# joshspeagle/brutus

Hardware: AMD Instinct MI355X
Metric: stars/sec at 750k-model x 12-band grid; achieved HBM GB/s vs peak (higher is better)
Workload: dtype f64; 1 GPU; configs[1]: 750k-model x 12-band grid, Av-only solve (rvlim=(3.32,3.32)), no parallax; grid = synth.make_mist_like_grid (lattice-ordered like the MIST grid files); grid_generator=mist_like, nmodel=750000, nfilt=12, sub_batch=128, selected_models_last_sub_batch=44670752, streams_per_gpu=3, parallelism=stars sharded, 1 rank(s), no data-path collective

## Files before the change

### brutus_amd/csrc/brutus_kernels.hip

```cpp

#include <hip/hip_runtime.h>
#include <math.h>
#include <stdint.h>
#include <string.h>

#include <atomic>
#include <vector>

#include "../../include/brutus_amd.h"
#include "../../include/brutus_amd_debug.h"

#include "host.hpp"
#include "common.hpp"
#include "fastmath.hpp"
#include "grid_kernels.hpp"
#include "fit_kernels.hpp"
#include "fit2_kernels.hpp"
#include "cut_kernels.hpp"

namespace {

struct ResBlock {
    enum { SELECTED, DERIVED, CANDIDATES, NTOTALS = 4, NUNCONV = 4, NCTR = 8, ZEROED = NUNCONV + NCTR };
    int64_t *totals;
    int32_t *k1, *k2, *n_unconv, *ctr;
    ResBlock(int64_t *base, int nstar) : totals(base), k1((int32_t *)(base + NTOTALS)), k2(k1 + nstar),
                                         n_unconv(k2 + nstar), ctr(n_unconv + NUNCONV) {}
    static size_t bytes(int nstar) { return sizeof(int64_t) * NTOTALS + sizeof(int32_t) * (2 * (size_t)nstar + ZEROED); }
};

struct Workspace {
    Planes pl;
    StarPrep *stars;
    double *part;
    double *vmax_lnlp;
    int32_t *k1;
    int32_t *k2;
    int32_t *n_unconv;
    int64_t *counts;
    int64_t *offsets;
    int32_t *ids;
    int32_t *ids2;
    int32_t *ctr;
    int32_t *hot;
    int64_t *res;
    int32_t *kfix;
    double *thr_cull, *maxsurv, *thr_sel;
    int32_t *surv_idx;
    int64_t *surv_off;
    int64_t *coffsets;
    int64_t *dcounts, *doffsets;
    int64_t *der_off;
    int32_t *wbase_surv, *wbase_der;
    ItemGeom *items_surv, *items_der;
    int32_t *bandn;
    unsigned long long *mask, *dmask;
    unsigned long long *smask;
    double *step_st, *lnprob_st;
    Star32 *s32;
    float *lnlp32, *lnpr32;
    float *part32, *st32;
    int32_t *status, *ids_all;
    double *nomA, *nomB, *candS;
    float *aud;
    StarPrep *stars_tmp;
    size_t part_doubles;
    size_t bytes;
};

Workspace carve(char *base, int64_t nmodel, int nstar, bool fit) {
    Workspace w{};
    Carver cv(base);
    const size_t pairs = (size_t)nstar * (size_t)nmodel;
    const int64_t ntile = pad_models(nmodel) / TILE;
    w.pl.nmodel = nmodel;
    w.stars = (StarPrep *)cv.take(sizeof(StarPrep) * nstar);
    w.part_doubles = (size_t)ntile * (size_t)(nstar * 2 * KCAP > 1024 ? nstar * 2 * KCAP : 1024);
    w.part = (double *)cv.take(sizeof(double) * w.part_doubles);
    w.stars_tmp = (StarPrep *)cv.take(sizeof(StarPrep));
    w.vmax_lnlp = (double *)cv.take(sizeof(double) * nstar);
    w.k1 = (int32_t *)cv.take(sizeof(int32_t) * nstar);
    w.k2 = (int32_t *)cv.take(sizeof(int32_t) * nstar);
    w.n_unconv = (int32_t *)cv.take(sizeof(int32_t) * 4);
    w.counts = (int64_t *)cv.take(sizeof(int64_t) * nstar * NCHUNK);
    w.offsets = (int64_t *)cv.take(sizeof(int64_t) * nstar * NCHUNK);
    if (!fit) {
        w.pl.lnlp = (double *)cv.take_big(sizeof(double) * pairs);
        w.pl.step = (double *)cv.take_big(sizeof(double) * pairs);
    } else {
        w.ids = (int32_t *)cv.take(sizeof(int32_t) * nstar);
        w.ids2 = (int32_t *)cv.take(sizeof(int32_t) * nstar);
        w.res = (int64_t *)cv.take(ResBlock::bytes(nstar));
        if (base) {
            const ResBlock res(w.res, nstar);
            w.k1 = res.k1;
            w.k2 = res.k2;
            w.n_unconv = res.n_unconv;
            w.ctr = res.ctr;
        }
        w.kfix = (int32_t *)cv.take(sizeof(int32_t) * nstar);
        w.thr_cull = (double *)cv.take(sizeof(double) * nstar);
        w.maxsurv = (double *)cv.take(sizeof(double) * nstar);
        w.thr_sel = (double *)cv.take(sizeof(double) * nstar);
        w.surv_off = (int64_t *)cv.take(sizeof(int64_t) * (nstar + 1));
        w.der_off = (int64_t *)cv.take(sizeof(int64_t) * (nstar + 1));
        w.coffsets = (int64_t *)cv.take(sizeof(int64_t) * nstar * NCHUNK);
        w.dcounts = (int64_t *)cv.take(sizeof(int64_t) * nstar * NCHUNK);
        w.doffsets = (int64_t *)cv.take(sizeof(int64_t) * nstar * NCHUNK);
        w.wbase_surv = (int32_t *)cv.take(sizeof(int32_t) * ((size_t)NCHUNK * nstar + 1));
        w.wbase_der = (int32_t *)cv.take(sizeof(int32_t) * ((size_t)NCHUNK * nstar + 1));
        {
            const size_t nit = (size_t)nstar * ((size_t)(pad_models(nmodel) / TILE) + NCHUNK);
            w.items_surv = (ItemGeom *)cv.take(sizeof(ItemGeom) * nit);
            w.items_der = (ItemGeom *)cv.take(sizeof(ItemGeom) * nit);
        }
        w.bandn = (int32_t *)cv.take(sizeof(int32_t) * (size_t)NCHUNK * nstar);
        const size_t words = (size_t)nstar * (size_t)(pad_models(nmodel) / 64);
        w.mask = (unsigned long long *)cv.take_big(sizeof(unsigned long long) * words);
        w.dmask = (unsigned long long *)cv.take_big(sizeof(unsigned long long) * words);
        w.smask = (unsigned long long *)cv.take_big(sizeof(unsigned long long) * words);
        const size_t nblk2 = (size_t)(ntile + F2_T - 1) / F2_T;
        w.s32 = (Star32 *)cv.take(sizeof(Star32) * nstar);
        w.part32 = (float *)cv.take(sizeof(float) * nblk2 * nstar * NV32);
        w.hot = (int32_t *)cv.take(sizeof(int32_t) * nblk2 * nstar);
        w.st32 = (float *)cv.take(sizeof(float) * nstar * NV32);
        w.status = (int32_t *)cv.take(sizeof(int32_t) * nstar);
        w.ids_all = (int32_t *)cv.take(sizeof(int32_t) * nstar);
        w.nomA = (double *)cv.take(sizeof(double) * nstar);
        w.nomB = (double *)cv.take(sizeof(double) * nstar);
        w.candS = (double *)cv.take(sizeof(double) * nstar);
        w.aud = (float *)cv.take(sizeof(float) * nstar * 4);
        w.lnlp32 = (float *)cv.take_big(sizeof(float) * pairs);
        w.lnpr32 = (float *)cv.take_big(sizeof(float) * pairs);
        w.surv_idx = (int32_t *)cv.take_big(sizeof(int32_t) * pairs);
        w.step_st = (double *)cv.take_big(sizeof(double) * pairs);
        w.lnprob_st = (double *)cv.take_big(sizeof(double) * pairs);
    }
    w.bytes = align_big(cv.off) + (base ? 0 : (size_t)4 << 20);
    return w;
}

int make_params(const brutus_params *in, DevParams &p) {
    if (!in) return fail(BRUTUS_EINVAL, "params is NULL");
    if (!(in->init_thresh > 0.) || !(in->ltol_subthresh > 0.))
        return fail(BRUTUS_EINVAL, "thresholds must be positive");
    if (in->init_thresh > in->ltol_subthresh)
        return fail(BRUTUS_EINVAL,
                    "The initial threshold must be smaller than or equal to the "
                    "final threshold applied to be useful!");
    p.avmin = in->avlim[0];
    p.avmax = in->avlim[1];
    p.rvmin = in->rvlim[0];
    p.rvmax = in->rvlim[1];
    p.av_mean = in->av_gauss[0];
    p.av_ivar = 1. / (in->av_gauss[1] * in->av_gauss[1]);
    p.rv_mean = in->rv_gauss[0];
    p.rv_ivar = 1. / (in->rv_gauss[1] * in->rv_gauss[1]);
    p.mtol = 2.5 * in->ltol;
    p.ltol = in->ltol;
    p.ln_init = log(in->init_thresh);
    p.ln_sub = log(in->ltol_subthresh);
    p.ln_wt = in->wt_thresh > 0. ? log(in->wt_thresh) : -INFINITY;
    p.a_reg = 1. / (0.05 * 0.05);
    p.r_reg = 1. / (0.1 * 0.1);
    p.dim_prior = in->dim_prior ? 1 : 0;
    return 0;
}

template <int NB>
int probe_k1_deep(const float *grid, int64_t nmodel, int star, const DevParams &p, int max_iter,
                  Workspace &w, int32_t *k1_out, hipStream_t st, const double *av_init = nullptr,
                  const double *rv_init = nullptr) {
    const int64_t nmodel_pad = pad_models(nmodel);
    const int ntile = (int)(nmodel_pad / TILE);
    HIP_TRY(hipMemcpyAsync(w.stars_tmp, w.stars + star, sizeof(StarPrep), hipMemcpyDeviceToDevice, st));
    const int cap = (int)(w.part_doubles / ((size_t)ntile * 2));
    for (int kmax = 16;; kmax *= 2) {
        if (kmax > max_iter) kmax = max_iter;
        if (kmax > cap) kmax = cap;
        hipLaunchKernelGGL(k_mag_stats<NB>, dim3(ntile, 1), dim3(TILE), 0, st, grid, nmodel,
                           nmodel_pad, 1, w.stars_tmp, p, kmax, w.part, av_init, rv_init);
        hipLaunchKernelGGL(k_k1_deep_decide, dim3(1), dim3(256), 0, st, ntile, kmax, w.part,
                           p.ln_init, w.k1 + star);
        HIP_TRY(hipMemcpyAsync(k1_out, w.k1 + star, sizeof(int32_t), hipMemcpyDeviceToHost, st));
        HIP_TRY(hipStreamSynchronize(st));
        if (*k1_out > 0) return 0;
        if (kmax >= max_iter || kmax >= cap)
            return fail(BRUTUS_ENOCONV, "magnitude phase of star %d not converged after %d sweeps",
// ... 58 lines not shown
                           w.part, p.ln_sub, (double *)nullptr, w.k2, w.n_unconv);
        HIP_TRY(hipMemcpyAsync(&h_unconv, w.n_unconv, sizeof(int32_t), hipMemcpyDeviceToHost, st));
        HIP_TRY(hipStreamSynchronize(st));
        if (h_unconv == 0) break;
        if (iter >= max_iter)
            return fail(BRUTUS_ENOCONV, "flux phase not converged after %d iterations for %d star(s)",
                        iter, h_unconv);
        ++iter;
    }

    tm.begin("k_finalize");
    hipLaunchKernelGGL(k_finalize, dim3(ntile, nstar), blk, 0, st, nmodel, nstar, w.stars, p,
                       w.vmax_lnlp, w.pl);
    tm.end();
    if (h_k1) HIP_TRY(hipMemcpyAsync(h_k1, w.k1, sizeof(int32_t) * nstar, hipMemcpyDeviceToHost, st));
    if (h_k2) HIP_TRY(hipMemcpyAsync(h_k2, w.k2, sizeof(int32_t) * nstar, hipMemcpyDeviceToHost, st));
    HIP_TRY(hipGetLastError());
    return 0;
}

int dispatch_pipeline(int nb, const float *grid, int64_t nmodel, int nstar, const DevParams &p,
                      int max_iter, Workspace &w, int32_t *h_k1, int32_t *h_k2,
                      hipStream_t st, Timer &tm, const double *av_init, const double *rv_init) {
    int rc = 0;
    if (with_nb(nb, GridBands{}, [&](auto NB) {
            rc = run_pipeline<decltype(NB)::value>(grid, nmodel, nstar, p, max_iter, w, h_k1, h_k2, st, tm, av_init, rv_init);
        }))
        return rc;
    return fail(BRUTUS_EINVAL, "unsupported band count %d", nb);
}

constexpr int BRUTUS_RETRY_HOSTDRIVEN = -1000;
std::atomic<long long> g_fit_calls{0}, g_fit_retries{0};
constexpr int FS_TILES_PER_BLOCK = 8, PERSIST_BLOCKS = 4096, CONT_BLOCKS = 2048, TOP_BLOCKS = 1024;

struct FitCall {
    const float *grid;
    int64_t nmodel, nmodel_pad;
    int ntile, nblkx;
    int nfilt, nstar;
    DevParams p;
    int max_iter;
    Workspace w;
    RecPlanes rec;
    int64_t capacity;
    int32_t *d_rec_idx, *d_rec_slot;
    int64_t *d_rec_off;
    int32_t *h_k1, *h_k2;
    int64_t *h_counts;
    hipStream_t st;
    Timer tm;
    int flux_rounds = 4;
    bool list_fast = true;
    int list_run = -LIST_RUN;
    bool audited = false;
    float *aud = nullptr;
};

inline bool rv_pinned(const DevParams &p) { return p.rvmin == p.rvmax && p.rv_mean == p.rvmin; }

P32 make_p32(const DevParams &p, int nfilt) {
    return P32{(float)p.avmin, (float)p.avmax, (float)p.rvmin, (float)p.rvmax, (float)p.av_mean, (float)p.av_ivar,
               (float)p.rv_mean, (float)p.rv_ivar, (float)(p.mtol * 1.002 + 1e-4), (float)(p.mtol * 0.998 - 1e-4),
               p.dim_prior, nfilt};
}

template <int NB, bool RVF>
int launch_pre32(FitCall &c, const int32_t *list, int nrun, const int32_t *nrun_dev, int accept,
                 int32_t *ctr, bool two_sweeps) {
    constexpr int G = 4;
    const Workspace &w = c.w;
    const P32 q = make_p32(c.p, c.nfilt);
    const int use_mfma = env_int("BRUTUS_PRE32_MFMA", 0);
    const int min_stars = env_int("BRUTUS_PRE32_STAR_LANES_MIN", 32);
    const bool lanes_are_stars = brutus_i_pre32s_bands(NB) && two_sweeps && nrun >= min_stars &&
                                 env_int("BRUTUS_PRE32_STAR_LANES", 1) != 0;
    c.tm.begin("k_pre32");
    if (lanes_are_stars) {
        if (brutus_i_pre32s_launch(NB, use_mfma, RVF ? 1 : 0, c.grid, c.nmodel, c.nmodel_pad, c.nstar, nrun, list,
                                   w.s32, &q, w.lnlp32, w.lnpr32, w.part32, c.st))
            return fail(BRUTUS_EHIP, "star-lane float32 pass: launch failed");
    } else {
        hipLaunchKernelGGL((k_pre32<NB, RVF, G>), dim3(8 * ((c.nblkx + 7) / 8) * ((nrun + G - 1) / G)),
                           dim3(TILE), 0, c.st, c.grid, c.nmodel, c.nmodel_pad, c.nstar, nrun, list, w.s32, q,
                           w.kfix, c.ntile, w.lnlp32, w.lnpr32, w.part32, nrun_dev);
    }
    c.tm.end();
    hipLaunchKernelGGL(k_pre_decide, dim3(nrun), dim3(256), 0, c.st, c.nblkx, c.nstar, list, w.part32,
                       w.s32, (float)c.p.ln_init, RVF ? 1 : 0, w.kfix, accept, w.st32, w.k1, w.status,
                       w.nomA, ctr, w.ids2, w.ids, nrun_dev);
    HIP_TRY(hipGetLastError());
    return 0;
}

template <int NB, bool RVF>
int pre32_all_stars(FitCall &c) { return launch_pre32<NB, RVF>(c, c.w.ids_all, c.nstar, nullptr, 0, c.w.ctr, true); }
template <int NB, bool RVF>
int pre32_redo_on_device(FitCall &c) { return launch_pre32<NB, RVF>(c, c.w.ids, c.nstar, c.w.ctr + 1, 1, nullptr, false); }
template <int NB, bool RVF>
int pre32_host_list(FitCall &c, const std::vector<int32_t> &ids, const std::vector<int32_t> &kfix, int accept) {
    const int nrun = (int)ids.size();
    HIP_TRY(hipMemcpyAsync(c.w.ids, ids.data(), sizeof(int32_t) * nrun, hipMemcpyHostToDevice, c.st));
    HIP_TRY(hipMemcpyAsync(c.w.kfix, kfix.data(), sizeof(int32_t) * c.nstar, hipMemcpyHostToDevice, c.st));
    bool two_sweeps = true;
    if (!RVF)
        for (int k = 0; k < nrun && two_sweeps; ++k) two_sweeps = kfix[ids[k]] == 2;
// ... 56 lines not shown
    const Workspace &w = c.w;
    if (c.aud) HIP_TRY(hipMemsetAsync(w.aud, 0, sizeof(float) * c.nstar * 4, c.st));
    c.h_counts[0] = c.h_counts[1] = c.h_counts[2] = 0;
    hipLaunchKernelGGL(k_prep32, dim3(c.nstar), dim3(64), 0, c.st, c.nstar, w.stars,
                       (float)env_double("BRUTUS_EPS_SCALE", 1.0), c.p.dim_prior, w.s32,
                       CallInit{w.ids_all, w.kfix, w.k2, w.n_unconv, ResBlock::ZEROED});
    return 0;
}

template <int NB, bool RVF>
int classify_on_device(FitCall &c) {
    if (int rc = pre32_all_stars<NB, RVF>(c)) return rc;
    if (int rc = k1probe_device_list<NB, RVF>(c)) return rc;
    if (!RVF)
        if (int rc = pre32_redo_on_device<NB, RVF>(c)) return rc;
    return 0;
}

template <int NB, bool RVF>
int classify_on_host(FitCall &c) {
    Workspace &w = c.w;
    const int nstar = c.nstar;
    std::vector<int32_t> ids(nstar), kfix(nstar, 2), k1(nstar, 0), status(nstar, 0);
    for (int s = 0; s < nstar; ++s) ids[s] = s;
    if (int rc = pre32_host_list<NB, RVF>(c, ids, kfix, 0)) return rc;
    HIP_TRY(hipMemcpyAsync(k1.data(), w.k1, sizeof(int32_t) * nstar, hipMemcpyDeviceToHost, c.st));
    HIP_TRY(hipMemcpyAsync(status.data(), w.status, sizeof(int32_t) * nstar, hipMemcpyDeviceToHost, c.st));
    HIP_TRY(hipStreamSynchronize(c.st));
    std::vector<int32_t> probe, redo;
    for (int s = 0; s < nstar; ++s) {
        if (status[s] == 1) redo.push_back(s);
        if (status[s] == 2) probe.push_back(s);
    }
    if (!probe.empty()) {
        if (int rc = k1probe_host_list<NB, RVF>(c, probe)) return rc;
        HIP_TRY(hipMemcpyAsync(k1.data(), w.k1, sizeof(int32_t) * nstar, hipMemcpyDeviceToHost, c.st));
        HIP_TRY(hipStreamSynchronize(c.st));
        for (int s : probe) {
            if (k1[s] == 0)
                if (int rc = probe_k1_deep<NB>(c.grid, c.nmodel, s, c.p, c.max_iter, w, &k1[s], c.st)) return rc;
            if (k1[s] > c.max_iter)
                return fail(BRUTUS_ENOCONV, "magnitude phase of star %d needs %d sweeps (max_iter %d)", s,
                            k1[s], c.max_iter);
            kfix[s] = k1[s];
            if (!RVF && k1[s] != 2) redo.push_back(s);
        }
    }
    for (int s : redo) kfix[s] = k1[s];
    if (!redo.empty())
        if (int rc = pre32_host_list<NB, RVF>(c, redo, kfix, 1)) return rc;
    return 0;
}

template <int NB, bool RVF>
void cull_candidates(FitCall &c) {
    const Workspace &w = c.w;
    const int nstar = c.nstar;
    const dim3 blk(TILE);
    c.tm.begin("k_top");
    hipLaunchKernelGGL(k_hot_list, dim3(nstar), dim3(256), 0, c.st, c.nblkx, nstar, 0, w.part32, w.nomA,
                       (const double *)nullptr, w.s32, (double *)nullptr, w.part, w.hot, w.ctr + 4);
    hipLaunchKernelGGL((k_top1<NB, RVF>), dim3(TOP_BLOCKS), blk, 0, c.st, c.grid, c.nmodel, c.nmodel_pad, nstar,
                       w.stars, c.p, w.k1, c.ntile, 0, w.lnlp32, w.nomA, w.hot, w.ctr + 4, w.part, c.aud);
    c.tm.end();
    hipLaunchKernelGGL(k_top_decide, dim3(nstar), dim3(256), 0, c.st, c.nblkx, nstar, w.ids_all, 0, w.part,
                       w.s32, c.p.ln_init, (const double *)nullptr, w.thr_cull, w.candS);
    c.tm.begin("k_surv_compact");
    if (!c.list_fast)
        hipLaunchKernelGGL(k_cmp_count32, dim3(NCHUNK, nstar), blk, 0, c.st, c.nmodel, c.ntile, w.lnlp32, w.candS,
                           w.counts, w.smask);
    else if (c.nmodel % 4 == 0)
        hipLaunchKernelGGL(k_cmp_count32_live<true>, dim3(NCHUNK, nstar), blk, 0, c.st, c.nmodel, c.ntile, nstar,
                           w.lnlp32, w.part32, w.candS, w.counts, w.smask);
    else
        hipLaunchKernelGGL(k_cmp_count32_live<false>, dim3(NCHUNK, nstar), blk, 0, c.st, c.nmodel, c.ntile, nstar,
                           w.lnlp32, w.part32, w.candS, w.counts, w.smask);
    const OffsetsJob job{w.counts, w.coffsets, w.surv_off, w.wbase_surv, w.res + ResBlock::CANDIDATES};
    hipLaunchKernelGGL(k_offsets, dim3(2), dim3(OFF_T), 0, c.st, nstar, job, job);
    hipLaunchKernelGGL(k_items, dim3((NCHUNK * nstar + 255) / 256), dim3(256), 0, c.st, nstar, w.wbase_surv,
                       w.coffsets, w.surv_off, w.items_surv);
    hipLaunchKernelGGL(k_cmp_scatter, dim3(NCHUNK, nstar), blk, 0, c.st, c.nmodel, c.ntile, w.smask,
                       w.coffsets, (int64_t)nstar * c.nmodel, w.surv_idx);
    c.tm.end();
}

enum class Asked { HostAfterFirstFlux, DeviceCandidates, WholeCall };
int capacity_verdict(const FitCall &c, Asked when, int64_t ncand, int64_t nder) {
    int64_t *n = c.h_counts;
    if (when != Asked::WholeCall) {
        if (ncand <= c.capacity) return 0;
        n[1] = ncand;
        n[2] = when == Asked::HostAfterFirstFlux
                   ? 2 * ncand
                   : ncand + (nder > 0 ? nder : ncand);
        return fail(BRUTUS_ENOMEM, "record buffer too small: %lld candidate slots, capacity %lld",
                    (long long)ncand, (long long)c.capacity);
    }
    n[1] = ncand;
    n[2] = ncand + nder;
    if (n[2] > c.capacity)
        return fail(BRUTUS_ENOMEM, "record buffer too small: %lld slots needed, capacity %lld",
                    (long long)n[2], (long long)c.capacity);
    return 0;
}

template <int NB, bool RVF>
void flux_on_device(FitCall &c) {
    const Workspace &w = c.w;
    for (int r = 0; r <= c.flux_rounds; ++r) {
        c.tm.begin(r == 0 ? "k_fflux" : "k_fflux_cont");
        if (r == 0) fflux_open<NB, RVF>(c);
        else fflux_continue_device<NB, RVF>(c, r, w.n_unconv + ((r - 1) & 1));
        c.tm.end();
        hipLaunchKernelGGL(k_fflux_decide, dim3(c.nstar), dim3(256), 0, c.st, c.nstar, w.wbase_surv, w.part,
                           c.p.ln_sub, w.k2, w.maxsurv, w.n_unconv + (r & 1), w.ids, w.n_unconv + ((r + 1) & 1));
    }
}

template <int NB, bool RVF>
int flux_on_host(FitCall &c, int64_t *ncand) {
    const Workspace &w = c.w;
    const int nstar = c.nstar;
    HIP_TRY(hipMemcpyAsync(ncand, w.surv_off + nstar, sizeof(int64_t), hipMemcpyDeviceToHost, c.st));
    int32_t h_unconv = 0;
    int iter = 2;
    std::vector<int32_t> k2s(nstar), act;
    for (int first = 1;; first = 0) {
        HIP_TRY(hipMemsetAsync(w.n_unconv, 0, sizeof(int32_t), c.st));
        c.tm.begin(first ? "k_fflux" : "k_fflux_cont");
        if (first) fflux_open<NB, RVF>(c);
        else fflux_continue_host<NB, RVF>(c, (int)act.size());
        c.tm.end();
        hipLaunchKernelGGL(k_fflux_decide, dim3(nstar), dim3(256), 0, c.st, nstar, w.wbase_surv, w.part,
                           c.p.ln_sub, w.k2, w.maxsurv, w.n_unconv, (int32_t *)nullptr, (int32_t *)nullptr);
        HIP_TRY(hipMemcpyAsync(&h_unconv, w.n_unconv, sizeof(int32_t), hipMemcpyDeviceToHost, c.st));
        HIP_TRY(hipMemcpyAsync(k2s.data(), w.k2, sizeof(int32_t) * nstar, hipMemcpyDeviceToHost, c.st));
        HIP_TRY(hipStreamSynchronize(c.st));
        if (first)
            if (int rc = capacity_verdict(c, Asked::HostAfterFirstFlux, *ncand, 0)) return rc;
        if (h_unconv == 0) return 0;
        if (iter >= c.max_iter)
            return fail(BRUTUS_ENOCONV, "flux phase not converged after %d iterations for %d star(s)",
                        iter, h_unconv);
        ++iter;
        act.clear();
        for (int s = 0; s < nstar; ++s)
            if (k2s[s] >= 0) act.push_back(s);
        HIP_TRY(hipMemcpyAsync(w.ids, act.data(), sizeof(int32_t) * act.size(), hipMemcpyHostToDevice, c.st));
    }
}

template <int NB, bool RVF>
void select_and_derive(FitCall &c) {
    const Workspace &w = c.w;
    const int nstar = c.nstar;
    const dim3 blk(TILE);
    c.tm.begin("k_top");
    hipLaunchKernelGGL(k_hot_list, dim3(nstar), dim3(256), 0, c.st, c.nblkx, nstar, 1, w.part32,
                       (const double *)nullptr, w.maxsurv, w.s32, w.nomB, w.part, w.hot, w.ctr + 5);
    hipLaunchKernelGGL((k_top1<NB, RVF>), dim3(TOP_BLOCKS), blk, 0, c.st, c.grid, c.nmodel, c.nmodel_pad, nstar,
                       w.stars, c.p, w.k1, c.ntile, 1, w.lnpr32, w.nomB, w.hot, w.ctr + 5, w.part,
                       c.aud ? c.aud + nstar : nullptr);
    c.tm.end();
    hipLaunchKernelGGL(k_top_decide, dim3(nstar), dim3(256), 0, c.st, c.nblkx, nstar, w.ids_all, 1, w.part,
                       w.s32, c.p.ln_wt, w.maxsurv, w.thr_sel, (double *)nullptr);
    c.tm.begin("k_sel_classify");
    if (c.list_fast && c.nmodel % 4 == 0)
        hipLaunchKernelGGL(k_sel_classify_live, dim3(NCHUNK, nstar), blk, 0, c.st, c.nmodel, c.ntile, nstar, w.s32,
                           w.lnpr32, w.part32, w.candS, w.lnprob_st, w.surv_off, w.thr_sel, w.counts, w.mask, w.dcounts,
                           w.dmask, w.surv_idx, w.bandn);
    else
        hipLaunchKernelGGL(k_sel_classify, dim3(NCHUNK, nstar), blk, 0, c.st, c.nmodel, c.ntile, w.s32, w.lnpr32,
                           w.lnprob_st, w.surv_off, w.thr_sel, w.counts, w.mask, w.dcounts, w.dmask, w.surv_idx, w.bandn);
    c.tm.end();
    c.tm.begin("k_sel_band");
    hipLaunchKernelGGL((k_sel_band<NB, RVF>), dim3(NCHUNK / SB_C, nstar, SB_Z), blk, 0, c.st, c.grid, c.nmodel,
                       c.nmodel_pad, c.ntile, w.stars, c.p, w.k1, w.lnpr32, w.thr_sel, w.surv_idx, w.bandn,
                       w.counts, w.mask, w.dcounts, w.dmask, c.aud ? c.aud + 2 * nstar : nullptr);
    c.tm.end();
    c.tm.begin("k_select");
    const OffsetsJob sel{w.counts, w.offsets, c.d_rec_off, nullptr, w.res + ResBlock::SELECTED};
    const OffsetsJob der{w.dcounts, w.doffsets, w.der_off, w.wbase_der, w.res + ResBlock::DERIVED};
    hipLaunchKernelGGL(k_offsets, dim3(4), dim3(OFF_T), 0, c.st, nstar, sel, der);
    hipLaunchKernelGGL(k_items, dim3((NCHUNK * nstar + 255) / 256), dim3(256), 0, c.st, nstar, w.wbase_der,
                       w.doffsets, w.der_off, w.items_der);
    hipLaunchKernelGGL(k_rec_index, dim3(NCHUNK, nstar), blk, 0, c.st, c.nmodel, c.ntile, nstar, w.mask, w.dmask,
                       w.smask, w.offsets, w.doffsets, w.coffsets, w.surv_off, c.capacity, c.d_rec_idx,
                       c.d_rec_slot, w.surv_idx);
    c.tm.end();
    c.tm.begin("k_derive");
    hipLaunchKernelGGL((k_derive<NB, RVF>), dim3(PERSIST_BLOCKS), blk, 0, c.st, c.grid, c.nmodel_pad, nstar,
                       w.stars, c.p, w.k1, w.surv_idx, w.wbase_der, w.items_der, w.surv_off, c.rec, c.list_run);
    c.tm.end();
}

int read_results(FitCall &c, std::vector<int64_t> &h_res) {
    h_res.resize((ResBlock::bytes(c.nstar) + sizeof(int64_t) - 1) / sizeof(int64_t));
    HIP_TRY(hipMemcpyAsync(h_res.data(), c.w.res, ResBlock::bytes(c.nstar), hipMemcpyDeviceToHost, c.st));
    HIP_TRY(hipGetLastError());
    HIP_TRY(hipStreamSynchronize(c.st));
    const ResBlock res(h_res.data(), c.nstar);
    c.h_counts[0] = res.totals[ResBlock::SELECTED];
    if (c.h_k1) memcpy(c.h_k1, res.k1, sizeof(int32_t) * c.nstar);
    if (c.h_k2) memcpy(c.h_k2, res.k2, sizeof(int32_t) * c.nstar);
    return 0;
}

template <int NB, bool RVF>
int run_fit(FitCall &c, bool device_driven) {
    int64_t ncand = 0;
    std::vector<int64_t> h_res;
    if (int rc = start_call(c)) return rc;
    if (int rc = device_driven ? classify_on_device<NB, RVF>(c) : classify_on_host<NB, RVF>(c)) return rc;
    cull_candidates<NB, RVF>(c);
    if (device_driven)
        flux_on_device<NB, RVF>(c);
    else if (int rc = flux_on_host<NB, RVF>(c, &ncand))
        return rc;
    select_and_derive<NB, RVF>(c);
    if (int rc = read_results(c, h_res)) return rc;
    const ResBlock res(h_res.data(), c.nstar);
    const int64_t nder = res.totals[ResBlock::DERIVED];
    if (device_driven) {
        ncand = res.totals[ResBlock::CANDIDATES];
        if (int rc = capacity_verdict(c, Asked::DeviceCandidates, ncand, nder)) return rc;
        if (res.ctr[3] != 0 || res.n_unconv[c.flux_rounds & 1] != 0) return BRUTUS_RETRY_HOSTDRIVEN;
    }
    return capacity_verdict(c, Asked::WholeCall, ncand, nder);
}

int audit_verdict(const Workspace &w, int nstar, hipStream_t st) {
    std::vector<float> aud(4 * (size_t)nstar);
    std::vector<Star32> s32(nstar);
    HIP_TRY(hipMemcpyAsync(aud.data(), w.aud, sizeof(float) * aud.size(), hipMemcpyDeviceToHost, st));
    HIP_TRY(hipMemcpyAsync(s32.data(), w.s32, sizeof(Star32) * (size_t)nstar, hipMemcpyDeviceToHost, st));
    HIP_TRY(hipStreamSynchronize(st));
    static const char *what[3] = {"cull statistic", "first-cut statistic (maximum)", "first-cut statistic (band)"};
    for (int r = 0; r < 3; ++r)
        for (int s = 0; s < nstar; ++s)
            if (!(aud[(size_t)r * nstar + s] < s32[s].eps))
                return fail(BRUTUS_EPRECISION,
                            "float32 proof bound violated: star %d of the batch, %s: |float32 - float64| = %.3g "
                            "against eps = %.3g (BRUTUS_EPS_SCALE raises the bound; please report the input)",
                            s, what[r], (double)aud[(size_t)r * nstar + s], (double)s32[s].eps);
    return 0;
}

int dispatch_fit(int nb, FitCall &c) {
    const bool rvf = rv_pinned(c.p);
    const bool hostdriven = env_int("BRUTUS_FIT_HOSTDRIVEN", 0) != 0;
    const long long call_no = g_fit_calls.fetch_add(1);
    const int every = env_int("BRUTUS_AUDIT_EVERY", 64);
    c.audited = every > 0 && call_no % every == 0;
    c.aud = env_int("BRUTUS_AUDIT", 0) != 0 || c.audited ? c.w.aud : nullptr;
    c.flux_rounds = env_int("BRUTUS_FLUX_ROUNDS", 4);
    c.list_fast = env_int("BRUTUS_LIST_FAST", 1) != 0;
    c.list_run = env_int("BRUTUS_LIST_RUN", 0);
    if (c.list_run < 1 || c.list_run > 64) c.list_run = -LIST_RUN;
    if (brutus_i_pre32_layout(0) != (int)sizeof(Star32) || brutus_i_pre32_layout(1) != (int)sizeof(P32) ||
        brutus_i_pre32_layout(2) != F2_T || brutus_i_pre32_layout(3) != TILE || brutus_i_pre32_layout(4) != NV32)
        return fail(BRUTUS_EINVAL, "float32 pass: the library's translation units disagree on the Star32 / "
                                   "tile layout (built with different flags?)");
    int rc = 0;
    const bool built = with_nb(nb, FitBands{}, [&](auto NB) {
        constexpr int N = decltype(NB)::value;
        auto run = [&](bool device_driven) {
            return rvf ? run_fit<N, true>(c, device_driven) : run_fit<N, false>(c, device_driven);
        };
        rc = hostdriven ? BRUTUS_RETRY_HOSTDRIVEN : run(true);
        if (rc == BRUTUS_RETRY_HOSTDRIVEN) {
            if (!hostdriven) g_fit_retries.fetch_add(1);
            rc = run(false);
        }
        if (rc == 0 && c.audited) rc = audit_verdict(c.w, c.nstar, c.st);
    });
    if (built) return rc;
    if (nb > BRUTUS_MAX_FILT_FIT)
        return fail(BRUTUS_EINVAL, "brutus_fit_batch fits at most %d bands at once (%d given): take the full-grid "
                                   "outputs of brutus_loglike_batch and cut on them", BRUTUS_MAX_FILT_FIT, c.nfilt);
    return fail(BRUTUS_EINVAL, "unsupported band count %d", nb);
}

int check_common(int64_t nmodel, int nfilt, int nstar) {
    if (nmodel <= 0 || nmodel > (int64_t)1 << 31) return fail(BRUTUS_EINVAL, "bad nmodel");
    if (padded_nb(nfilt) < 0 || nfilt < 1)
        return fail(BRUTUS_EINVAL, "nfilt=%d unsupported (max %d)", nfilt, BRUTUS_MAX_FILT);
    if (nstar < 1 || nstar > BRUTUS_MAX_BATCH)
        return fail(BRUTUS_EINVAL, "nstar=%d outside [1, %d]", nstar, BRUTUS_MAX_BATCH);
    return 0;
}

int launch_prep(int nstar, int nfilt, const double *d_flux, const double *d_err,
                const uint8_t *d_mask, const double *d_par, const double *d_perr, int has_par,
                Workspace &w, int32_t *d_ndim, hipStream_t st) {
    hipLaunchKernelGGL(k_prep, dim3(nstar), dim3(64), 0, st, nstar, nfilt, d_flux,
                       d_err, d_mask, d_par, d_perr, (d_par && d_perr) ? has_par : 0, w.stars,
                       d_ndim);
    HIP_TRY(hipGetLastError());
    return 0;
}

void fix_k2(int32_t *h_k2, int nstar) {
    if (!h_k2) return;
    for (int s = 0; s < nstar; ++s)
        if (h_k2[s] < 0) h_k2[s] = -h_k2[s] - 1;
}

}

// ... 200 lines not shown
        tm.collect();
        return fail(BRUTUS_ENOMEM, "record buffer too small: %lld rows needed, capacity %lld",
                    (long long)(rec_base + total), (long long)capacity);
    }
    CutPlanes pl;
    pl.v[0] = d_lnl;
    pl.v[1] = d_chi2;
    pl.v[2] = d_scale;
    pl.v[3] = d_av;
    pl.v[4] = d_rv;
    for (int q = 0; q < 6; ++q) pl.v[5 + q] = d_icov + (size_t)q * nstar * nmodel;
    tm.begin("cut_scatter");
    if (vec)
        hipLaunchKernelGGL(k_cut_scatter<true>, grid, block, 0, st, nmodel, w.stride, span, nstar,
                           w.lnprob, w.thr, w.counts, w.offsets, d_lnl, pl, next, d_ext_labels,
                           d_ext_par, capacity, d_rec_idx, d_rec_slot, d_rec_vals);
    else
        hipLaunchKernelGGL(k_cut_scatter<false>, grid, block, 0, st, nmodel, w.stride, span, nstar,
                           w.lnprob, w.thr, w.counts, w.offsets, d_lnl, pl, next, d_ext_labels,
                           d_ext_par, capacity, d_rec_idx, d_rec_slot, d_rec_vals);
    tm.end();
    HIP_TRY(hipGetLastError());
    HIP_TRY(hipStreamSynchronize(st));
    tm.collect();
    return 0;
}

int brutus_debug_fit_stats(int64_t *calls, int64_t *repeated) {
    if (calls) *calls = g_fit_calls.load();
    if (repeated) *repeated = g_fit_retries.load();
    return 0;
}

int brutus_debug_copy(void *d_workspace, size_t workspace_bytes, int64_t nmodel, int nfilt, int nstar,
                      int which, void *d_dst, size_t nbytes, void *stream) {
    if (int rc = check_common(nmodel, nfilt, nstar)) return rc;
    if (!d_workspace || !d_dst) return fail(BRUTUS_EINVAL, "NULL pointer");
    Workspace w = carve((char *)d_workspace, nmodel, nstar, true);
    if (w.bytes > workspace_bytes) return fail(BRUTUS_ENOMEM, "workspace too small");
    const size_t plane = (size_t)nstar * (size_t)nmodel;
    const void *src = nullptr;
    size_t have = 0;
    switch (which) {
        case 2: src = w.lnlp32; have = 4 * plane; break;
        case 3: src = w.lnpr32; have = 4 * plane; break;
        case 4: src = w.aud; have = 4 * (size_t)nstar * 4; break;
        case 5: src = w.s32; have = sizeof(Star32) * (size_t)nstar; break;
        case 6: src = w.thr_cull; have = 8 * (size_t)nstar; break;
        case 7: src = w.thr_sel; have = 8 * (size_t)nstar; break;
        case 8: src = w.st32; have = 4 * (size_t)nstar * NV32; break;
        case 9: src = w.status; have = 4 * (size_t)nstar; break;
        case 10: src = w.part32; have = 4 * (size_t)((pad_models(nmodel) / TILE + F2_T - 1) / F2_T) * nstar * NV32; break;
        case 11: src = w.candS; have = 8 * (size_t)nstar; break;
        default: return fail(BRUTUS_EINVAL, "unknown array %d", which);
    }
    if (nbytes > have) return fail(BRUTUS_EINVAL, "array %d holds %zu bytes, %zu requested", which, have, nbytes);
    HIP_TRY(hipMemcpyAsync(d_dst, src, nbytes, hipMemcpyDeviceToDevice, (hipStream_t)stream));
    return 0;
}

int brutus_debug_sizeof_star32(void) { return (int)sizeof(Star32); }

int brutus_debug_pre32_time(void *d_workspace, size_t workspace_bytes, const float *d_grid_soa,
                            int64_t nmodel, int nfilt, int nstar, const brutus_params *params,
                            int form, int reps, float *h_ms, void *stream) {
    if (int rc = check_common(nmodel, nfilt, nstar)) return rc;
    if (!d_workspace || !d_grid_soa || !h_ms || reps < 1) return fail(BRUTUS_EINVAL, "bad arguments");
    DevParams p;
    if (int rc = make_params(params, p)) return rc;
    Workspace w = carve((char *)d_workspace, nmodel, nstar, true);
    if (w.bytes > workspace_bytes) return fail(BRUTUS_ENOMEM, "workspace too small");
    const int nb = brutus_padded_filters(nfilt);
    if (!brutus_i_pre32s_bands(nb)) return fail(BRUTUS_EINVAL, "no star-lane pass for %d bands", nb);
    const bool rvf = rv_pinned(p);
    const P32 q = make_p32(p, nfilt);
    hipStream_t st = (hipStream_t)stream;
    hipEvent_t a, b;
    HIP_TRY(hipEventCreate(&a));
    HIP_TRY(hipEventCreate(&b));
    for (int k = 0; k < reps + 1; ++k) {
        if (k == 1) HIP_TRY(hipEventRecord(a, st));
        if (brutus_i_pre32s_launch(nb, form, rvf ? 1 : 0, d_grid_soa, nmodel, pad_models(nmodel), nstar, nstar,
                                   w.ids_all, w.s32, &q, w.lnlp32, w.lnpr32, w.part32, st))
            return fail(BRUTUS_EHIP, "star-lane float32 pass: launch failed");
    }
    HIP_TRY(hipEventRecord(b, st));
    HIP_TRY(hipEventSynchronize(b));
    float ms = 0.f;
    HIP_TRY(hipEventElapsedTime(&ms, a, b));
    *h_ms = ms / reps;
    (void)hipEventDestroy(a);
    (void)hipEventDestroy(b);
    return 0;
}

}
```

### brutus_amd/csrc/fit2_kernels.hpp

```cpp
#pragma once

#include "fit_kernels.hpp"
#include "pre32_types.hpp"

namespace {

static_assert(PS_TILE == TILE && PS_NBMAX == NBMAX, "pre32_types.hpp and common.hpp disagree");

struct CallInit {
    int32_t *ids_all, *kfix, *k2, *counters;
    int ncounters;
};
__global__ void __launch_bounds__(64)
k_prep32(int nstar, const StarPrep *__restrict__ stars, float eps_scale, int dim_prior,
         Star32 *__restrict__ out, CallInit init) {
    static_assert(NBMAX <= 64, "one lane per band");
    __shared__ double s_a[NBMAX], s_b[NBMAX], s_c[NBMAX];
    __shared__ double s_gbar, s_D;
    __shared__ int s_bad;
    const int s = blockIdx.x, j = threadIdx.x;
    if (s >= nstar) return;
    if (init.ids_all && j == 0) {
        init.ids_all[s] = s;
        init.kfix[s] = 2;
// ... 413 lines not shown
        double a_, c_;
        if (K > 0) gram_sweep_rf(Gm, sp.S, p, av, a_, c_);
    } else {
        Gram Gm;
        gram_init<NB>(t.c, sp, Gm);
        for (int k = 0; k < K; ++k) {
            double a_, b_, c_;
            gram_sweep(Gm, sp.S, p, av, rv, a_, b_, c_);
        }
    }
}

template <int NB, bool RVF, bool FULL>
__device__ __forceinline__ void mle_at(const Tile64<NB, RVF> &t, const StarPrep &sp,
                                       const DevParams &p, double av, double rv,
                                       const double *__restrict__ tbl, Mle &m) {
    if constexpr (RVF) mle_fast_rf<NB, true, FULL ? 2 : 0>(t.c, t.R, t.F0, sp, p, av, tbl, m);
    else mle_fast<NB, true, FULL ? 2 : 0>(t.c, t.F0, sp, p, av, rv, tbl, m);
}

__device__ __forceinline__ void audit(float *__restrict__ aud, int s, float f32v, double f64v,
                                      double thr) {
    if (aud && f64v > thr - 12. && f32v == f32v) {
        const float d = fabsf((float)(f64v - (double)f32v));
        atomicMax(reinterpret_cast<int *>(aud + s), __float_as_int(d));
    }
}

__device__ __forceinline__ int64_t mword(int s, int ntile, int t, int w) {
    return (int64_t)s * (4 * ntile) + (int64_t)t * 4 + w;
}

__global__ void __launch_bounds__(256)
k_hot_list(int nblkx, int nstar, int mode, const float *__restrict__ part32,
           const double *__restrict__ nomA, const double *__restrict__ maxsurv,
           const Star32 *__restrict__ s32, double *__restrict__ nomB, double *__restrict__ part,
           int32_t *__restrict__ hot, int32_t *__restrict__ nhot) {
    const int s = blockIdx.x;
    double nm;
    if (mode == 0) {
        nm = nomA[s];
    } else {
        nm = maxsurv[s] - (double)s32[s].eps;
        if (threadIdx.x == 0) nomB[s] = nm;
    }
    for (int b = threadIdx.x; b < nblkx; b += blockDim.x) {
        const float *pp = part32 + ((int64_t)b * nstar + s) * NV32;
        const bool is_hot = !((double)pp[6 + mode] < nm) || pp[9] > 0.f;
        if (is_hot) hot[atomicAdd(nhot, 1)] = b * BRUTUS_MAX_BATCH + s;
        else part[(int64_t)b * nstar + s] = -INFINITY;
    }
}

template <int NB, bool RVF>
__global__ void __launch_bounds__(TILE, top_waves(NB))
k_top1(const float *__restrict__ grid, int64_t nmodel, int64_t nmodel_pad, int nstar,
       const StarPrep *__restrict__ stars, DevParams p, const int32_t *__restrict__ k1, int ntile,
       int mode, const float *__restrict__ plane32, const double *__restrict__ nom,
       const int32_t *__restrict__ hot, const int32_t *__restrict__ nhot,
       double *__restrict__ part, float *__restrict__ aud) {
    __shared__ double slot[4];
    __shared__ double s_tbl[64];
    const int n = *nhot;
    if ((int)blockIdx.x >= n) return;
    stage_exp_table(s_tbl);
    __syncthreads();
    const int lane = threadIdx.x & 63;
    for (int e = blockIdx.x; e < n; e += gridDim.x) {
        const int entry = hot[e];
        const int b = entry / BRUTUS_MAX_BATCH, s = entry - b * BRUTUS_MAX_BATCH;
        const int t0 = b * F2_T, t1 = min(ntile, t0 + F2_T);
        const StarPrep &sp = stars[s];
        const double nm_s = nom[s];
        const int K = k1[s];
        float v[F2_T];
#pragma unroll
        for (int u = 0; u < F2_T; ++u) {
            const int64_t i = (int64_t)(t0 + u) * TILE + threadIdx.x;
            v[u] = plane32[(int64_t)s * nmodel + (i < nmodel ? i : nmodel - 1)];
        }
        double mx = -INFINITY;
#pragma unroll
        for (int u = 0; u < F2_T; ++u) {
            const int64_t i = (int64_t)(t0 + u) * TILE + threadIdx.x;
            bool mine = t0 + u < t1 && i < nmodel && !((double)v[u] < nm_s);
            if (mode == 1 && mine) mine = !surv_is(v[u]);
            if (__ballot(mine) == 0ull) continue;
            Tile64<NB, RVF> tl;
            tile_load<NB, RVF>(grid, nmodel_pad, i, p.rv_mean, tl);
            double av, rv;
            mag_phase<NB, RVF>(tl, sp, p, K, av, rv);
            Mle m;
            mle_at<NB, RVF, false>(tl, sp, p, av, rv, s_tbl, m);
            double val;
            if (mode == 0) val = cull_stat(sp, m);
            else val = first_cut_lnprob(sp, final_lnl<false>(sp, p, m.chi2, false), m.scale, m.i00);
            if (mine) audit(aud, s, v[u], val, nm_s);
            if (mine && val == val) mx = val > mx ? val : mx;
        }
        block_max_store(mx, slot, part + (int64_t)b * nstar + s);
    }
}

__global__ void k_top_decide(int nblkx, int nstar, const int32_t *__restrict__ star_ids, int mode,
                             const double *__restrict__ part, const Star32 *__restrict__ s32,
                             double ln_thr, const double *__restrict__ maxsurv,
// ... 440 lines not shown
```

### brutus_amd/csrc/fit_kernels.hpp

```cpp
#pragma once

#include "common.hpp"
#include "fastmath.hpp"
#include "grid_kernels.hpp"

namespace {


struct Gram {
    double ua, ub, uy, aa, ab, bb, ay, by, yy;
};

template <int NB>
__device__ __forceinline__ void gram_init(const Coef<NB> &c, const StarPrep &sp, Gram &G) {
    double ua = 0., ub = 0., uy = 0., aa = 0., ab = 0., bb = 0., ay = 0., by = 0., yy = 0.;
#pragma unroll
    for (int j = 0; j < NB; ++j) {
        const double w = sp.iW[j];
        const double a = (double)c.r0[j], b = (double)c.dr[j];
        const double y = sp.g[j] - (double)c.m[j];
        const double aw = a * w, bw = b * w, yw = y * w;
        ua += aw;
        ub += bw;
        uy += yw;
// ... 716 lines not shown
}

typedef float f32x4 __attribute__((ext_vector_type(4)));
template <int NB>
struct RowRegs {
    f32x4 q[3 * NB / 4];
};
template <int NB>
__device__ __forceinline__ void gather_row(const float *__restrict__ grid, int64_t nmodel_pad,
                                           int64_t i, RowRegs<NB> &r) {
    const f32x4 *row =
        reinterpret_cast<const f32x4 *>(grid + (int64_t)3 * NB * nmodel_pad + i * (3 * NB));
#pragma unroll
    for (int q = 0; q < 3 * NB / 4; ++q) r.q[q] = row[q];
}
template <int NB>
__device__ __forceinline__ void row_to_coef(const RowRegs<NB> &r, Coef<NB> &c) {
    float t[3 * NB];
#pragma unroll
    for (int q = 0; q < 3 * NB / 4; ++q) {
        t[4 * q] = r.q[q].x;
        t[4 * q + 1] = r.q[q].y;
        t[4 * q + 2] = r.q[q].z;
        t[4 * q + 3] = r.q[q].w;
    }
#pragma unroll
    for (int j = 0; j < NB; ++j) {
        c.m[j] = t[3 * j];
        c.r0[j] = t[3 * j + 1];
        c.dr[j] = t[3 * j + 2];
    }
}
template <int NB>
__device__ __forceinline__ void landed(RowRegs<NB> &r) {
#pragma unroll
    for (int q = 0; q < 3 * NB / 4; ++q) {
        f32x4 t = r.q[q];
        asm volatile("" : "+v"(t) : : "memory");
        r.q[q] = t;
    }
}
__device__ __forceinline__ void landed(int32_t &x) {
    int32_t t = x;
    asm volatile("" : "+v"(t) : : "memory");
    x = t;
}

struct RecPlanes {
    double *vals;
    int64_t cap;
    __device__ __forceinline__ double *plane(int v) const { return vals + (int64_t)v * cap; }
};

template <int NB, bool RVF, bool FIRST>
__global__ void __launch_bounds__(TILE, fflux_waves(NB, FIRST))
k_fflux(const float *__restrict__ grid, int64_t nmodel, int64_t nmodel_pad, int nstar,
        const StarPrep *__restrict__ stars, DevParams p, const int32_t *__restrict__ k1,
        const int32_t *__restrict__ k2state, const int32_t *__restrict__ cand_idx,
        const int64_t *__restrict__ cand_off, const int32_t *__restrict__ wbase,
        const ItemGeom *__restrict__ items, RecPlanes rec, double *__restrict__ step_st,
        double *__restrict__ lnprob_st, double *__restrict__ part, float *__restrict__ surv32,
        const double *__restrict__ thr_cull, const int32_t *__restrict__ act, int nact,
        const int32_t *__restrict__ nact_dev, int run) {
    if (!FIRST && nact_dev) nact = *nact_dev;
    if (!FIRST && nact <= 0) return;
    __shared__ double s_tbl[64];
    stage_exp_table(s_tbl);
    __syncthreads();
    constexpr bool WIDE = wide_bands(NB);
    __shared__ double s_F[WIDE ? NB * TILE : 1];
    const LdsColumn Fc = (LdsColumn)s_F + (WIDE ? threadIdx.x : 0);
    constexpr int niter = FIRST ? 2 : 1;
    int s_nxt = 0;
    auto lane_model = [&](int item) -> int32_t {
        const ItemGeom ig = items[item < 0 ? 0 : item];
        s_nxt = ig.s;
        const int64_t q = ig.q0 + threadIdx.x;
        const int64_t last = ig.q0 + ig.n - 1;
        return cand_idx[q < last ? q : last];
    };
    double *__restrict__ r_lnl = rec.plane(0), *__restrict__ r_chi2 = rec.plane(1),
                        *__restrict__ r_scale = rec.plane(2), *__restrict__ r_av = rec.plane(3),
                        *__restrict__ r_rv = rec.plane(4);
    auto walk = [&](auto &wk) {
    int32_t i_nxt = lane_model(wk.item);
    constexpr bool PER_STAR = FIRST && NB <= 12;
    double aL = -INFINITY, aT = -INFINITY, aM = -INFINITY;
    while (!wk.done()) {
        const int item = wk.item;
        wk.next();
        const ItemGeom ig = items[item];
        const int s = ig.s;
        const int32_t i_me = i_nxt;
        i_nxt = lane_model(wk.item);
        if (k2state[s] < 0) {
            landed(i_nxt);
            continue;
        }
        const StarPrep &sp = stars[s];
        const int64_t q = ig.q0 + threadIdx.x;
        const bool live = (int)threadIdx.x < ig.n && q < rec.cap;
        double L = -INFINITY, T = -INFINITY, M = -INFINITY;
        bool go = live;
        const int64_t i = i_me;
        const int64_t o = (int64_t)s * nmodel + i;
        if (!FIRST && live) go = surv_is(surv32[o]);
        Mle m;
        double o_lnl = 0., o_lnprob = 0., o_av = 0., o_rv = 0., o_step = 0.;
        bool store = false;
        if (go) {
            Coef<NB> c;
            gather_coef<NB>(grid, nmodel_pad, i, c);
            double F0[WIDE ? 1 : NB];
#ifdef BRUTUS_F0_FROM_TABLE
            if constexpr (!WIDE) load_F0<NB>(grid, nmodel_pad, i, F0);
#else
            if constexpr (!WIDE) compute_F0_tbl<NB>(c, s_tbl, F0);
#endif
            double av, rv, step, lnl_old;
            double R[RVF && !WIDE ? NB : 1];
            if constexpr (RVF && !WIDE) coef_R<NB>(c, p.rv_mean, R);
            if constexpr (FIRST) {
                av = p.av_mean;
                rv = p.rv_mean;
                const int K = k1[s];
                if constexpr (RVF) {
                    GramR G;
                    if constexpr (WIDE) gram_init_rf_wide<NB>(c, p.rv_mean, sp, G);
                    else gram_init_rf<NB>(c, R, sp, G);
                    for (int k = 0; k < K; ++k) {
                        double a_, c_;
                        gram_sweep_rf(G, sp.S, p, av, a_, c_);
                    }
                } else {
                    Gram G;
                    gram_init<NB>(c, sp, G);
                    for (int k = 0; k < K; ++k) {
                        double a_, b_, c_;
                        gram_sweep(G, sp.S, p, av, rv, a_, b_, c_);
                    }
                }
                step = 1.0;
                lnl_old = -BIG;
            } else {
                av = r_av[q];
                rv = RVF ? p.rv_mean : r_rv[q];
                step = step_st[q];
                lnl_old = -0.5 * r_chi2[q];
            }
            mle_list<NB, RVF, false>(c, R, F0, Fc, sp, p, av, rv, s_tbl, m);
            if constexpr (FIRST) {
                go = cull_stat(sp, m) > thr_cull[s];
                if (go) surv32[o] = surv_tag(q - cand_off[s]);
            }
            double lnl_new = lnl_old, dl = 0.;
            for (int it = 0; go && it < niter; ++it) {
                double dav = (m.a_num + (p.av_mean - av) * p.av_ivar) / (m.a_ss + p.av_ivar) * step;
                if (dav < p.avmin - av) dav = p.avmin - av;
                if (dav > p.avmax - av) dav = p.avmax - av;
                av += dav;
                if constexpr (RVF) {
                    if (it + 1 < niter) mle_list<NB, RVF, false>(c, R, F0, Fc, sp, p, av, rv, s_tbl, m);
                    else mle_list<NB, RVF, true>(c, R, F0, Fc, sp, p, av, rv, s_tbl, m);
                } else {
                    double drv = (m.r_num + (p.rv_mean - rv) * p.rv_ivar) / (m.r_ss + p.rv_ivar) * step;
                    if (drv < p.rvmin - rv) drv = p.rvmin - rv;
                    if (drv > p.rvmax - rv) drv = p.rvmax - rv;
                    rv += drv;
                    constexpr bool SHORT_FIRST = NB != 16;
                    if (SHORT_FIRST && it + 1 < niter) mle_list<NB, RVF, false>(c, R, F0, Fc, sp, p, av, rv, s_tbl, m);
                    else mle_list<NB, RVF, true>(c, R, F0, Fc, sp, p, av, rv, s_tbl, m);
                }
                lnl_new = -0.5 * m.chi2;
                dl = fabs(lnl_new - lnl_old);
                if (lnl_new < lnl_old) step /= 1.2;
                lnl_old = lnl_new;
            }
            if (go) {
                o_lnl = final_lnl<RVF>(sp, p, m.chi2, true);
                o_lnprob = first_cut_lnprob(sp, o_lnl, m.scale, m.i00);
                o_av = av;
                o_rv = rv;
                o_step = step;
                M = o_lnprob;
                if (lnl_new == lnl_new) {
                    L = lnl_new;
                    if (dl > p.ltol) T = lnl_new;
                }
            }
            store = go;
        }
        landed(i_nxt);
        if (store) {
#define FF_ST(p, x) __builtin_nontemporal_store((x), (p) + q)
            FF_ST(r_lnl, o_lnl);
            FF_ST(r_chi2, m.chi2);
            FF_ST(r_scale, m.scale);
            FF_ST(r_av, o_av);
            if constexpr (!RVF) FF_ST(r_rv, o_rv);
            FF_ST(rec.plane(5), m.i00);
            FF_ST(rec.plane(6), m.i01);
            FF_ST(rec.plane(7), m.i02);
            FF_ST(rec.plane(8), m.i11);
            FF_ST(rec.plane(9), m.i12);
            FF_ST(rec.plane(10), m.i22);
            FF_ST(step_st, o_step);
            FF_ST(lnprob_st, o_lnprob);
#undef FF_ST
        }
        if constexpr (PER_STAR) {
            aL = L > aL ? L : aL;
            aT = T > aT ? T : aT;
            aM = M > aM ? M : aM;
            L = T = M = -INFINITY;
            if (wk.done() || s_nxt != s) {
                L = wave_max_dpp(aL);
                T = wave_max_dpp(aT);
                M = wave_max_dpp(aM);
                aL = aT = aM = -INFINITY;
            }
        } else {
            L = wave_max_dpp(L);
            T = wave_max_dpp(T);
            M = wave_max_dpp(M);
        }
        if ((threadIdx.x & 63) == 0) {
            double *out = part + ((int64_t)item * (TILE / 64) + (threadIdx.x >> 6)) * 3;
            out[0] = L;
            out[1] = T;
            out[2] = M;
        }
    }
    };
    if constexpr (FIRST) {
        ItemWalk wk;
        wk.init(wbase, nstar, blockIdx.x & 7, blockIdx.x >> 3, (gridDim.x + 7 - (blockIdx.x & 7)) >> 3, run);
        walk(wk);
    } else {
        const int nunit = NCHUNK * nact * CONT_P;
        for (int unit = blockIdx.x; unit < nunit; unit += gridDim.x) {
            SegWalk wk;
            wk.init(wbase, nstar, act, nact, unit);
            walk(wk);
        }
    }
}

__global__ void k_fflux_decide(int nstar, const int32_t *__restrict__ wbase,
                               const double *__restrict__ part, double ln_sub,
                               int32_t *__restrict__ k2state, double *__restrict__ maxsurv,
                               int32_t *__restrict__ n_unconv, int32_t *__restrict__ act,
                               int32_t *__restrict__ zero_next) {
    __shared__ double sm[3][4];
    const int s = blockIdx.x;
    if (zero_next && s == 0 && threadIdx.x == 0) *zero_next = 0;
    if (k2state[s] < 0) return;
    double v[3] = {-INFINITY, -INFINITY, -INFINITY};
    const int per = TILE / 64;
    {
// ... 219 lines not shown
```

Baseline: 39680 stars/s.

## Screen hot-block list per model row and store step as shrink count

Adds a screened hot-list kernel that, for blocks whose partial summary says hot, rescans the per-model float plane to confirm at least one model clears the threshold before listing the block for k_top1. Blocks that fail are marked -inf and skipped. Separately, the per-pair step state is stored as a 16-bit count of step shrinks instead of a double, cutting write and read traffic in the flux kernel. The FIRST pass infers the count from the step value, assuming at most two shrinks. The screen adds extra reads of the lnlp/lnpr plane and more launched blocks per star.

```diff
diff --git a/brutus_amd/csrc/brutus_kernels.hip b/brutus_amd/csrc/brutus_kernels.hip
--- a/brutus_amd/csrc/brutus_kernels.hip
+++ b/brutus_amd/csrc/brutus_kernels.hip
@@ -56,7 +56,8 @@
     int32_t *bandn;
     unsigned long long *mask, *dmask;
     unsigned long long *smask;
-    double *step_st, *lnprob_st;
+    uint16_t *step_st;
+    double *lnprob_st;
     Star32 *s32;
     float *lnlp32, *lnpr32;
     float *part32, *st32;
@@ -133,7 +134,7 @@
         w.lnlp32 = (float *)cv.take_big(sizeof(float) * pairs);
         w.lnpr32 = (float *)cv.take_big(sizeof(float) * pairs);
         w.surv_idx = (int32_t *)cv.take_big(sizeof(int32_t) * pairs);
-        w.step_st = (double *)cv.take_big(sizeof(double) * pairs);
+        w.step_st = (uint16_t *)cv.take_big(sizeof(double) * pairs);
         w.lnprob_st = (double *)cv.take_big(sizeof(double) * pairs);
     }
     w.bytes = align_big(cv.off) + (base ? 0 : (size_t)4 << 20);
@@ -298,6 +299,7 @@
     Timer tm;
     int flux_rounds = 4;
     bool list_fast = true;
+    bool top1_screen = true;
     int list_run = -LIST_RUN;
     bool audited = false;
     float *aud = nullptr;
@@ -460,14 +462,26 @@
     return 0;
 }
 
+void launch_hot_list(const FitCall &c, int mode, int32_t *nhot) {
+    const Workspace &w = c.w;
+    const double *nomA = mode == 0 ? w.nomA : nullptr, *maxsurv = mode == 0 ? nullptr : w.maxsurv;
+    double *nomB = mode == 0 ? nullptr : w.nomB;
+    if (c.top1_screen)
+        hipLaunchKernelGGL(k_hot_list_screened, dim3(c.nstar, HOT_SPLIT), dim3(HOT_T), 0, c.st, c.nblkx, c.nstar, mode,
+                           c.nmodel, w.part32, mode == 0 ? w.lnlp32 : w.lnpr32, nomA, maxsurv, w.s32, nomB, w.part,
+                           w.hot, nhot);
+    else
+        hipLaunchKernelGGL(k_hot_list, dim3(c.nstar), dim3(256), 0, c.st, c.nblkx, c.nstar, mode, w.part32, nomA,
+                           maxsurv, w.s32, nomB, w.part, w.hot, nhot);
+}
+
 template <int NB, bool RVF>
 void cull_candidates(FitCall &c) {
     const Workspace &w = c.w;
     const int nstar = c.nstar;
     const dim3 blk(TILE);
     c.tm.begin("k_top");
-    hipLaunchKernelGGL(k_hot_list, dim3(nstar), dim3(256), 0, c.st, c.nblkx, nstar, 0, w.part32, w.nomA,
-                       (const double *)nullptr, w.s32, (double *)nullptr, w.part, w.hot, w.ctr + 4);
+    launch_hot_list(c, 0, w.ctr + 4);
     hipLaunchKernelGGL((k_top1<NB, RVF>), dim3(TOP_BLOCKS), blk, 0, c.st, c.grid, c.nmodel, c.nmodel_pad, nstar,
                        w.stars, c.p, w.k1, c.ntile, 0, w.lnlp32, w.nomA, w.hot, w.ctr + 4, w.part, c.aud);
     c.tm.end();
@@ -564,8 +578,7 @@
     const int nstar = c.nstar;
     const dim3 blk(TILE);
     c.tm.begin("k_top");
-    hipLaunchKernelGGL(k_hot_list, dim3(nstar), dim3(256), 0, c.st, c.nblkx, nstar, 1, w.part32,
-                       (const double *)nullptr, w.maxsurv, w.s32, w.nomB, w.part, w.hot, w.ctr + 5);
+    launch_hot_list(c, 1, w.ctr + 5);
     hipLaunchKernelGGL((k_top1<NB, RVF>), dim3(TOP_BLOCKS), blk, 0, c.st, c.grid, c.nmodel, c.nmodel_pad, nstar,
                        w.stars, c.p, w.k1, c.ntile, 1, w.lnpr32, w.nomB, w.hot, w.ctr + 5, w.part,
                        c.aud ? c.aud + nstar : nullptr);
@@ -663,6 +676,7 @@
     c.aud = env_int("BRUTUS_AUDIT", 0) != 0 || c.audited ? c.w.aud : nullptr;
     c.flux_rounds = env_int("BRUTUS_FLUX_ROUNDS", 4);
     c.list_fast = env_int("BRUTUS_LIST_FAST", 1) != 0;
+    c.top1_screen = env_int("BRUTUS_TOP1_SCREEN", 1) != 0;
     c.list_run = env_int("BRUTUS_LIST_RUN", 0);
     if (c.list_run < 1 || c.list_run > 64) c.list_run = -LIST_RUN;
     if (brutus_i_pre32_layout(0) != (int)sizeof(Star32) || brutus_i_pre32_layout(1) != (int)sizeof(P32) ||
@@ -969,6 +983,8 @@
         case 9: src = w.status; have = 4 * (size_t)nstar; break;
         case 10: src = w.part32; have = 4 * (size_t)((pad_models(nmodel) / TILE + F2_T - 1) / F2_T) * nstar * NV32; break;
         case 11: src = w.candS; have = 8 * (size_t)nstar; break;
+        case 12: src = w.nomA; have = 8 * (size_t)nstar; break;
+        case 13: src = w.nomB; have = 8 * (size_t)nstar; break;
         default: return fail(BRUTUS_EINVAL, "unknown array %d", which);
     }
     if (nbytes > have) return fail(BRUTUS_EINVAL, "array %d holds %zu bytes, %zu requested", which, have, nbytes);
diff --git a/brutus_amd/csrc/fit2_kernels.hpp b/brutus_amd/csrc/fit2_kernels.hpp
--- a/brutus_amd/csrc/fit2_kernels.hpp
+++ b/brutus_amd/csrc/fit2_kernels.hpp
@@ -489,6 +489,66 @@
     }
 }
 
+constexpr int HOT_SPLIT = 8, HOT_T = 256;
+__global__ void __launch_bounds__(HOT_T)
+k_hot_list_screened(int nblkx, int nstar, int mode, int64_t nmodel, const float *__restrict__ part32,
+                    const float *__restrict__ plane32, const double *__restrict__ nomA,
+                    const double *__restrict__ maxsurv, const Star32 *__restrict__ s32,
+                    double *__restrict__ nomB, double *__restrict__ part, int32_t *__restrict__ hot,
+                    int32_t *__restrict__ nhot) {
+    constexpr int CAP = 4 * HOT_T;
+    __shared__ int s_blk[CAP];
+    __shared__ int s_nb;
+    const int s = blockIdx.x;
+    double nm;
+    if (mode == 0) {
+        nm = nomA[s];
+    } else {
+        nm = maxsurv[s] - (double)s32[s].eps;
+        if (threadIdx.x == 0 && blockIdx.y == 0) nomB[s] = nm;
+    }
+    const float *__restrict__ row = plane32 + (int64_t)s * nmodel;
+    const int lane = threadIdx.x & 63;
+    for (int base = blockIdx.y; base < nblkx; base += CAP * HOT_SPLIT) {
+        if (threadIdx.x == 0) s_nb = 0;
+        __syncthreads();
+        for (int k = threadIdx.x; k < CAP; k += HOT_T) {
+            const int b = base + k * HOT_SPLIT;
+            if (b >= nblkx) break;
+            const float *pp = part32 + ((int64_t)b * nstar + s) * NV32;
+            const bool is_hot = !((double)pp[6 + mode] < nm) || pp[9] > 0.f;
+            if (is_hot) s_blk[atomicAdd(&s_nb, 1)] = b;
+            else part[(int64_t)b * nstar + s] = -INFINITY;
+        }
+        __syncthreads();
+        const int nb = s_nb;
+        for (int q = threadIdx.x >> 6; q < nb; q += HOT_T / 64) {
+            const int b = s_blk[q];
+            const int64_t i0 = (int64_t)b * (F2_T * TILE) + lane;
+            constexpr int U = F2_T * TILE / 64;
+            float v[U];
+#pragma unroll
+            for (int u = 0; u < U; ++u) {
+                const int64_t i = i0 + 64 * u;
+                v[u] = row[i < nmodel ? i : nmodel - 1];
+            }
+            bool any = false;
+#pragma unroll
+            for (int u = 0; u < U; ++u) {
+                bool mine = i0 + 64 * u < nmodel && !((double)v[u] < nm);
+                if (mode == 1 && mine) mine = !surv_is(v[u]);
+                any |= mine;
+            }
+            const bool listed = __ballot(any) != 0ull;
+            if (lane == 0) {
+                if (listed) hot[atomicAdd(nhot, 1)] = b * BRUTUS_MAX_BATCH + s;
+                else part[(int64_t)b * nstar + s] = -INFINITY;
+            }
+        }
+        __syncthreads();
+    }
+}
+
 template <int NB, bool RVF>
 __global__ void __launch_bounds__(TILE, top_waves(NB))
 k_top1(const float *__restrict__ grid, int64_t nmodel, int64_t nmodel_pad, int nstar,
diff --git a/brutus_amd/csrc/fit_kernels.hpp b/brutus_amd/csrc/fit_kernels.hpp
--- a/brutus_amd/csrc/fit_kernels.hpp
+++ b/brutus_amd/csrc/fit_kernels.hpp
@@ -792,13 +792,14 @@
     __device__ __forceinline__ double *plane(int v) const { return vals + (int64_t)v * cap; }
 };
 
+constexpr int STEP_SHRUNK_MAX = 65535;
 template <int NB, bool RVF, bool FIRST>
 __global__ void __launch_bounds__(TILE, fflux_waves(NB, FIRST))
 k_fflux(const float *__restrict__ grid, int64_t nmodel, int64_t nmodel_pad, int nstar,
         const StarPrep *__restrict__ stars, DevParams p, const int32_t *__restrict__ k1,
         const int32_t *__restrict__ k2state, const int32_t *__restrict__ cand_idx,
         const int64_t *__restrict__ cand_off, const int32_t *__restrict__ wbase,
-        const ItemGeom *__restrict__ items, RecPlanes rec, double *__restrict__ step_st,
+        const ItemGeom *__restrict__ items, RecPlanes rec, uint16_t *__restrict__ step_st,
         double *__restrict__ lnprob_st, double *__restrict__ part, float *__restrict__ surv32,
         const double *__restrict__ thr_cull, const int32_t *__restrict__ act, int nact,
         const int32_t *__restrict__ nact_dev, int run) {
@@ -846,7 +847,8 @@
         const int64_t o = (int64_t)s * nmodel + i;
         if (!FIRST && live) go = surv_is(surv32[o]);
         Mle m;
-        double o_lnl = 0., o_lnprob = 0., o_av = 0., o_rv = 0., o_step = 0.;
+        double o_lnl = 0., o_lnprob = 0., o_av = 0., o_rv = 0.;
+        int o_shrunk = 0, shrunk = 0;
         bool store = false;
         if (go) {
             Coef<NB> c;
@@ -885,7 +887,9 @@
             } else {
                 av = r_av[q];
                 rv = RVF ? p.rv_mean : r_rv[q];
-                step = step_st[q];
+                shrunk = step_st[q];
+                step = 1.0;
+                for (int k = 0; k < shrunk && step > 0.; ++k) step /= 1.2;
                 lnl_old = -0.5 * r_chi2[q];
             }
             mle_list<NB, RVF, false>(c, R, F0, Fc, sp, p, av, rv, s_tbl, m);
@@ -913,7 +917,10 @@
                 }
                 lnl_new = -0.5 * m.chi2;
                 dl = fabs(lnl_new - lnl_old);
-                if (lnl_new < lnl_old) step /= 1.2;
+                if (lnl_new < lnl_old) {
+                    step /= 1.2;
+                    if constexpr (!FIRST) shrunk = shrunk < STEP_SHRUNK_MAX ? shrunk + 1 : shrunk;
+                }
                 lnl_old = lnl_new;
             }
             if (go) {
@@ -921,7 +928,8 @@
                 o_lnprob = first_cut_lnprob(sp, o_lnl, m.scale, m.i00);
                 o_av = av;
                 o_rv = rv;
-                o_step = step;
+                if constexpr (FIRST) o_shrunk = step == 1.0 ? 0 : step == 1.0 / 1.2 ? 1 : 2;
+                else o_shrunk = shrunk;
                 M = o_lnprob;
                 if (lnl_new == lnl_new) {
                     L = lnl_new;
@@ -944,7 +952,7 @@
             FF_ST(rec.plane(8), m.i11);
             FF_ST(rec.plane(9), m.i12);
             FF_ST(rec.plane(10), m.i22);
-            FF_ST(step_st, o_step);
+            FF_ST(step_st, (uint16_t)o_shrunk);
             FF_ST(lnprob_st, o_lnprob);
 #undef FF_ST
         }
```

New measurement: 40560 stars/s, median of 6. 2.2% higher.
